# faasm/faabric

Hardware: AMD Instinct MI355X
Metric: MPI_Allreduce GB/s + batch-exec msgs/sec, 8-rank world at 1/2/4/8 MI355X (higher is better)
Workload: dtype fp32; 1 GPU; model=faabric composite: 256MB fp32 allreduce + 1MB alltoall + kvtouch batch, global_batch=128, parallelism=mpi1, allreduce_bytes=268435456, pingpong_bytes=0, kv_bytes=4096, full=False, snapshot_bytes_per_rank=0, snapshot_dirty=random-scattered 25pct, random-byte region, gpu=True

## Files before the change

### cpp/bindings/bindings_runtime.cpp

```cpp
#include <pybind11/functional.h>
#include <pybind11/pybind11.h>
#include <pybind11/stl.h>

#include "faabricamd/endpoint.h"
#include "faabricamd/executor.h"
#include "faabricamd/flat.h"
#include "faabricamd/hipipc.h"
#include "faabricamd/planner.h"
#include "faabricamd/ptp.h"
#include "faabricamd/runner.h"
#include "faabricamd/scheduler.h"
#include "faabricamd/snapshot.h"
#include "faabricamd/state.h"
#include "faabricamd/util.h"
#include "faabricamd/utilextras.h"
#include "faabricamd/dirty.h"
#include <hip/hip_runtime.h>

namespace py = pybind11;
using namespace faabricamd;

namespace faabricamd {
void registerBenchFunctions();
std::map<std::string, std::vector<uint8_t>> benchLastOutputs();
// ... 794 lines not shown
            PageAlignedBuffer buf;
            buf.resize(16 * 4096);
            tracker.startTracking(buf.data(), buf.size());
            buf.data()[2 * 4096 + 11] = 42;
            buf.data()[14 * 4096] = 7;
            tracker.stopTracking(buf.data(), buf.size());
            auto dirty = tracker.getDirtyPages(buf.data(), buf.size());
            int nDirty = 0;
            for (char d : dirty) {
                nDirty += d != 0;
            }
            ok = nDirty == 2 && dirty[2] == 1 && dirty[14] == 1;
        }
        return py::bool_(ok);
    });

    m.def("_selftest_softpte_tracker", []() -> py::object {
        if (!SoftPTEDirtyTracker::isAvailable()) {
            return py::none();
        }
        bool ok;
        {
            py::gil_scoped_release release;
            SoftPTEDirtyTracker tracker;
            PageAlignedBuffer buf;
            buf.resize(16 * 4096);
            std::memset(buf.data(), 1, buf.size());
            tracker.startTracking(buf.data(), buf.size());
            buf.data()[5 * 4096 + 3] = 42;
            buf.data()[12 * 4096] = 7;
            tracker.stopTracking(buf.data(), buf.size());
            auto dirty = tracker.getDirtyPages(buf.data(), buf.size());
            ok = dirty.size() == 16 && dirty[5] == 1 && dirty[12] == 1;
        }
        return py::bool_(ok);
    });

    m.def("_debug_runtime_sizes", [] {
        py::dict d;
        d["planner_app_results"] = Planner::get().debugAppResultsCount();
        d["planner_done_apps"] = Planner::get().debugDoneAppsCount();
        d["planner_in_flight"] = Planner::get().debugInFlightCount();
        d["broker_mappings"] = getPointToPointBroker().debugMappingsCount();
        d["broker_channels"] = getPointToPointBroker().debugChannelsCount();
        d["broker_send_seqs"] = getPointToPointBroker().debugSendSeqsCount();
        d["decision_cache"] = DecisionCache::get().size();
        return d;
    });
    m.def("_debug_dispatch_sizes", [] {
        py::dict d;
        d["idle_executors"] = Scheduler::get().debugIdleCount();
        d["planner_msg_index_apps"] = Planner::get().debugMsgIndexCount();
        d["planner_used_slots"] = Planner::get().debugUsedSlots();
        return d;
    });
    m.def("_debug_current_executor_id", [] {
        return ExecutorContext::get().getExecutor()->id;
    });
    m.def("_debug_set_message_result", [](const Message& msg) {
        auto copy = std::make_shared<Message>(msg);
        py::gil_scoped_release release;
        getPlannerClient().setMessageResult(copy);
    });
    m.def("_debug_kv_commit_stats", [] {
        KvCommitStats s = kvCommitStats();
        py::dict d;
        d["launches"] = s.launches;
        d["pages"] = s.pages;
        return d;
    });
    m.def("_debug_kv_sweep_bitmap",
          [](size_t nPages, const std::vector<uint64_t>& setBits) {
              size_t nWords = (nPages + 63) / 64;
              auto words = std::make_unique<std::atomic<uint64_t>[]>(
                std::max<size_t>(nWords, 1));
              for (size_t w = 0; w < nWords; w++) {
                  words[w].store(0);
              }
              for (uint64_t b : setBits) {
                  if (b >= nPages) {
                      throw FaabricException("bit beyond the bitmap");
                  }
                  words[b / 64].fetch_or(1ULL << (b % 64));
              }
              std::vector<uint32_t> pages(nPages);
              size_t n =
                kvSweepDirtyBitmap(words.get(), nPages, pages.data());
              pages.resize(n);
              std::vector<uint64_t> after(nWords);
              for (size_t w = 0; w < nWords; w++) {
                  after[w] = words[w].load();
              }
              return py::make_tuple(pages, after);
          },
          py::arg("n_pages"),
          py::arg("set_bits"));
    m.def("wait_batch_done",
          [](int32_t appId, int timeoutMs) {
              py::gil_scoped_release release;
              return getPlannerClient().waitBatchDone(appId, timeoutMs);
          },
          py::arg("app_id"),
          py::arg("timeout_ms") = 30000);
    m.def("set_bound_timeout",
          [](int ms) { getSystemConfig().boundTimeout = ms; });
    m.def("reap_stale_executors", [] {
        py::gil_scoped_release release;
        return Scheduler::get().reapStaleExecutors();
    });
    m.def("register_bench_functions", [] { registerBenchFunctions(); });
    m.def("bench_last_outputs", [] {
        py::dict d;
        for (const auto& [name, data] : benchLastOutputs()) {
            d[py::str(name)] =
              py::bytes((const char*)data.data(), data.size());
        }
        return d;
    });
    m.def("register_mpi_example_functions",
          [] { registerMpiExampleFunctions(); });

    m.def("execute_threads",
          [](const std::string& user,
             const std::string& function,
             int nThreads,
             const std::vector<std::tuple<uint32_t, size_t, int, int>>&
               regions,
             const py::bytes& inputData,
             bool elastic) {
              Executor* exec = ExecutorContext::get().getExecutor();
              std::string input = inputData;
              std::vector<std::pair<int32_t, int32_t>> results;
              {
                  py::gil_scoped_release release;
                  auto req = std::make_shared<BatchExecuteRequest>(
                    batchExecFactory(user, function, nThreads));
                  req->elasticScaleHint = elastic;
                  for (auto& m2 : req->messages) {
                      m2.inputData.assign(input.begin(), input.end());
                  }
                  std::vector<SnapshotMergeRegion> mr;
                  for (const auto& [off, len, dt, op] : regions) {
                      mr.emplace_back(off,
                                      len,
                                      (SnapshotDataType)dt,
                                      (SnapshotMergeOperation)op);
                  }
                  results = exec->executeThreads(req, mr);
              }
              py::list out;
              for (auto& [msgId, rv] : results) {
                  out.append(py::make_tuple(msgId, rv));
              }
              return out;
          },
          py::arg("user"),
          py::arg("function"),
          py::arg("n_threads"),
// ... 123 lines not shown
```

### cpp/include/faabricamd/executor.h

```cpp
#pragma once

#include <atomic>
#include <functional>
#include <memory>
#include <string>
#include <thread>
#include <vector>

#include "faabricamd/mailbox.h"
#include "faabricamd/messages.h"
#include "faabricamd/queue.h"
#include "faabricamd/dirty.h"
#include "faabricamd/snapshot.h"

namespace faabricamd {

class Executor;


class ExecutorContext
{
  public:
    static bool isSet();
    static void set(Executor* executor,
// ... 64 lines not shown
    std::vector<std::pair<int32_t, int32_t>> executeThreads(
      std::shared_ptr<BatchExecuteRequest> req,
      const std::vector<SnapshotMergeRegion>& mergeRegions);

    virtual int32_t executeTask(int threadPoolIdx,
                                int msgIdx,
                                std::shared_ptr<BatchExecuteRequest> req);

    virtual std::pair<uint8_t*, size_t> getMemoryView();
    virtual void setMemorySize(size_t newSize);
    void setDeviceMemorySize(size_t newSize);
    std::pair<uint8_t*, size_t> getDeviceMemoryView();
    bool hasDeviceArena() const { return deviceArena != nullptr; }
    virtual void restore(const std::string& snapshotKey);
    virtual void reset(Message& msg);
    virtual void flush();

    bool tryClaim();
    void claim();
    void releaseClaim();
    bool isClaimed() const { return claimed.load(); }
    using IdleExecutors = IdleList<std::shared_ptr<Executor>>;
    void setIdleList(std::shared_ptr<IdleExecutors> list)
    {
        idleList = std::move(list);
    }

    long getMillisSinceLastExec() const;
    void shutdown();

    std::string id;
    Message boundMsg;
    int gpuDevice = -1;

    void setThreadResult(Message& msg,
                         int32_t returnValue,
                         const std::string& key,
                         const std::vector<SnapshotDiffMsg>& diffs);

  protected:
    void threadPoolThread(int poolIdx);
    void handleTaskResult(Message& msg,
                          int32_t returnValue,
                          std::shared_ptr<BatchExecuteRequest> req,
                          bool isLastInBatch);

    int threadPoolSize = 0;
    using TaskMailbox = Mailbox<ExecutorTask>;
    std::vector<std::unique_ptr<TaskMailbox>> threadMailboxes;
    std::vector<std::thread> threadPoolThreads;
    std::unique_ptr<std::atomic<bool>[]> poolThreadUp;
    std::mutex threadsMx;
    void ensurePoolThreadLocked(int poolIdx);
    void postTask(int poolIdx, ExecutorTask&& task);

    std::shared_ptr<IdleExecutors> idleList;

    std::atomic<bool> claimed{ false };
    std::atomic<int64_t> lastExecMs{ 0 };

    std::string lastForkSnapshotKey;
    std::vector<std::string> lastForkRemoteHosts;
    void cleanupForkSnapshot();

    std::shared_ptr<std::atomic<int>> batchCounter;

    PageAlignedBuffer dummyMemory;

    uint8_t* deviceArena = nullptr;
    size_t deviceArenaSize = 0;
};

class ExecutorFactory
{
  public:
    virtual ~ExecutorFactory() = default;
    virtual std::shared_ptr<Executor> createExecutor(Message& msg)
    {
        return std::make_shared<Executor>(msg);
    }
    virtual void flushHost() {}
};

void setExecutorFactory(std::shared_ptr<ExecutorFactory> factory);
std::shared_ptr<ExecutorFactory> getExecutorFactory();

int32_t chainFunction(const std::string& user,
                      const std::string& function,
                      const std::vector<uint8_t>& input);
Message awaitChainedCall(int32_t msgId, int timeoutMs = 60000);

int32_t migrationPoint(const std::vector<uint8_t>& reentryInput);

}
```

### cpp/include/faabricamd/mailbox.h

```cpp
#pragma once

#include <atomic>
#include <climits>
#include <cstddef>
#include <cstdint>
#include <ctime>
#include <mutex>
#include <utility>
#include <vector>

#include <linux/futex.h>
#include <sys/syscall.h>
#include <unistd.h>

namespace faabricamd {

namespace detail {

inline void futexWait(std::atomic<uint32_t>* word,
                      uint32_t expected,
                      int timeoutMs)
{
    static_assert(sizeof(std::atomic<uint32_t>) == sizeof(uint32_t));
    struct timespec ts;
    struct timespec* tsp = nullptr;
    if (timeoutMs > 0) {
        ts.tv_sec = timeoutMs / 1000;
        ts.tv_nsec = (long)(timeoutMs % 1000) * 1000000L;
        tsp = &ts;
    }
    syscall(SYS_futex,
            reinterpret_cast<uint32_t*>(word),
            FUTEX_WAIT_PRIVATE,
            expected,
            tsp,
            nullptr,
            0);
}

inline void futexWake(std::atomic<uint32_t>* word, int n)
{
    syscall(SYS_futex,
            reinterpret_cast<uint32_t*>(word),
            FUTEX_WAKE_PRIVATE,
            n,
            nullptr,
            nullptr,
            0);
}

}

template<typename T, uint32_t SLOTS = 8>
class Mailbox
{
    static_assert(SLOTS >= 2 && (SLOTS & (SLOTS - 1)) == 0,
                  "SLOTS must be a power of two");

  public:
    Mailbox()
    {
        for (uint32_t i = 0; i < SLOTS; i++) {
            slots[i].seq.store(i, std::memory_order_relaxed);
        }
    }
    Mailbox(const Mailbox&) = delete;
    Mailbox& operator=(const Mailbox&) = delete;

    void post(T value)
    {
        uint32_t ticket = tail.fetch_add(1, std::memory_order_relaxed);
        Slot& s = slots[ticket & (SLOTS - 1)];
        uint32_t seen;
        while ((seen = s.seq.load(std::memory_order_acquire)) != ticket) {
            detail::futexWait(&s.seq, seen, 1);
        }
        s.value = std::move(value);
        s.seq.store(ticket + 1, std::memory_order_seq_cst);
        if (sleeping.load(std::memory_order_seq_cst) != 0) {
            detail::futexWake(&s.seq, INT_MAX);
        }
    }

    bool take(T& out, int timeoutMs)
    {
        Slot& s = slots[head & (SLOTS - 1)];
        uint32_t ready = head + 1;
        uint32_t seen = s.seq.load(std::memory_order_acquire);
        if (seen != ready) {
            struct timespec start;
            clock_gettime(CLOCK_MONOTONIC, &start);
            int leftMs = timeoutMs;
            while (true) {
                sleeping.store(1, std::memory_order_seq_cst);
                seen = s.seq.load(std::memory_order_seq_cst);
                if (seen != ready) {
                    detail::futexWait(&s.seq, seen, leftMs);
                    seen = s.seq.load(std::memory_order_acquire);
                }
                sleeping.store(0, std::memory_order_relaxed);
                if (seen == ready) {
                    break;
                }
                if (timeoutMs > 0) {
                    struct timespec now;
                    clock_gettime(CLOCK_MONOTONIC, &now);
                    int64_t goneMs =
                      (int64_t)(now.tv_sec - start.tv_sec) * 1000 +
                      (now.tv_nsec - start.tv_nsec) / 1000000;
                    if (goneMs >= timeoutMs) {
                        return false;
                    }
                    leftMs = (int)(timeoutMs - goneMs);
                }
            }
        }
        out = std::move(s.value);
        s.value = T();
        s.seq.store(head + SLOTS, std::memory_order_release);
        head++;
        return true;
    }

  private:
    struct alignas(64) Slot
    {
        std::atomic<uint32_t> seq{ 0 };
        T value{};
    };
    Slot slots[SLOTS];
    alignas(64) std::atomic<uint32_t> tail{ 0 };
    std::atomic<uint32_t> sleeping{ 0 };
    alignas(64) uint32_t head = 0;
};

template<typename T>
class IdleList
{
  public:
    void push(T value)
    {
        std::lock_guard<std::mutex> lock(mx);
        if (!closed) {
            entries.push_back(std::move(value));
        }
    }

    size_t popMany(size_t n, std::vector<T>& out)
    {
        std::lock_guard<std::mutex> lock(mx);
        size_t got = 0;
        while (got < n && !entries.empty()) {
            out.push_back(std::move(entries.back()));
            entries.pop_back();
            got++;
        }
        return got;
    }

    bool pop(T& out)
    {
        std::lock_guard<std::mutex> lock(mx);
        if (entries.empty()) {
            return false;
        }
        out = std::move(entries.back());
        entries.pop_back();
        return true;
    }

    size_t remove(const T& value)
    {
        std::lock_guard<std::mutex> lock(mx);
        size_t before = entries.size();
        size_t w = 0;
        for (size_t r = 0; r < entries.size(); r++) {
            if (!(entries[r] == value)) {
                if (w != r) {
                    entries[w] = std::move(entries[r]);
                }
                w++;
            }
        }
        entries.resize(w);
        return before - w;
    }

    void close()
    {
        std::vector<T> dropped;
        {
            std::lock_guard<std::mutex> lock(mx);
            closed = true;
            dropped.swap(entries);
        }
    }

    size_t size()
    {
        std::lock_guard<std::mutex> lock(mx);
        return entries.size();
    }

  private:
    std::mutex mx;
    std::vector<T> entries;
    bool closed = false;
};

}
```

### cpp/include/faabricamd/scheduler.h

```cpp
#pragma once

#include <memory>
#include <mutex>
#include <shared_mutex>
#include <unordered_map>
#include <vector>

#include "faabricamd/executor.h"
#include "faabricamd/messages.h"
#include "faabricamd/queue.h"
#include "faabricamd/transport.h"

namespace faabricamd {

enum class FunctionCalls : uint8_t
{
    ExecuteFunctions = 1,
    Flush = 2,
    SetMessageResult = 3,
    BatchDone = 4,
};

class Scheduler
{
  public:
    static Scheduler& get();

    void executeBatch(std::shared_ptr<BatchExecuteRequest> req);

    HostResources getThisHostResources();
    void setThisHostResources(const HostResources& res);

    int reapStaleExecutors();
    void startReaper();
    void stopReaper();

    std::shared_ptr<PendingMigration> checkForMigrationOpportunities(
      Message& msg,
      int32_t overwriteNewGroupId = 0);

    void flushLocally();
    void shutdown();
    void reset();

    std::vector<Message> getRecordedMessages();
    void clearRecordedMessages();

    size_t getExecutorCount();
    size_t debugIdleCount();

  private:
    Scheduler();

    struct WarmPool
    {
        std::vector<std::shared_ptr<Executor>> list;
        std::shared_ptr<Executor::IdleExecutors> idle =
          std::make_shared<Executor::IdleExecutors>();
    };

    std::shared_ptr<Executor> claimExecutor(Message& msg);
    void claimExecutors(BatchExecuteRequest& req,
                        std::vector<std::shared_ptr<Executor>>& execs,
                        std::vector<std::string>& errors);
    std::shared_ptr<Executor> createExecutorLocked(WarmPool& pool,
                                                   Message& msg);

    std::shared_mutex schedMx;
    std::unordered_map<std::string, std::unique_ptr<WarmPool>> executors;
    HostResources overriddenResources;
    bool resourcesOverridden = false;

    std::vector<Message> recordedMessages;

    class ReaperThread;
    std::shared_ptr<ReaperThread> reaper;
};

bool functionCallServerRunning();

class FunctionCallServer : public MessageEndpointServer
{
  public:
    FunctionCallServer();
    ~FunctionCallServer() override;
    void doAsyncRecv(uint8_t code,
                     const std::string& body,
                     uint32_t seq) override;
    std::string doSyncRecv(uint8_t code, const std::string& body) override;
};

class FunctionCallClient : public MessageEndpointClient
{
  public:
    explicit FunctionCallClient(const std::string& host);
    void executeFunctions(const BatchExecuteRequest& req);
    void setMessageResult(const Message& msg);
    void sendFlush();
    void batchDone(int32_t appId);
};

std::shared_ptr<FunctionCallClient> getFunctionCallClient(
  const std::string& host);

std::shared_ptr<FlagWaiter> batchDoneWaiterPrepare(int32_t appId);
void batchDoneWaiterDiscard(int32_t appId);
void signalBatchDone(int32_t appId);
void clearFunctionCallClients();

std::vector<std::pair<std::string, BatchExecuteRequest>>
getBatchRequestsSentMock();
void clearMockedFunctionCalls();

}
```

### cpp/src/executor.cpp

```cpp
#include "faabricamd/executor.h"
#include "faabricamd/utilextras.h"
#include "faabricamd/mpi.h"
#include "faabricamd/ops.h"
#include "faabricamd/planner.h"

#include <hip/hip_runtime.h>
#include "faabricamd/snapshot.h"
#include "faabricamd/util.h"

#include <algorithm>
#include <cstring>

namespace faabricamd {

void resultBatcherEnqueue(std::shared_ptr<Message> msg);


static thread_local std::shared_ptr<ExecutorContext> currentContext;

bool ExecutorContext::isSet()
{
    return currentContext != nullptr;
}

void ExecutorContext::set(Executor* executor,
                          std::shared_ptr<BatchExecuteRequest> req,
                          int msgIdx)
{
    auto ctx = std::make_shared<ExecutorContext>();
    ctx->executor = executor;
    ctx->req = std::move(req);
    ctx->msgIdx = msgIdx;
    currentContext = ctx;
}

void ExecutorContext::unset()
{
    currentContext = nullptr;
}

ExecutorContext& ExecutorContext::get()
{
    if (!currentContext) {
        throw FaabricException("no executor context set");
    }
    return *currentContext;
}

Message& ExecutorContext::getMsg()
{
    return req->messages.at(msgIdx);
}


FunctionRegistry& FunctionRegistry::get()
{
    static FunctionRegistry reg;
    return reg;
}

void FunctionRegistry::registerFunction(const std::string& user,
                                        const std::string& function,
                                        FaabricFunction fn)
{
    std::lock_guard<std::mutex> lock(mx);
    functions[user + "/" + function] = std::move(fn);
}

// ... 96 lines not shown
    std::lock_guard<std::mutex> lock(threadsMx);
    for (int i = 0; i < threadPoolSize; i++) {
        if (threadPoolThreads[i].joinable()) {
            ExecutorTask stopTask;
            stopTask.stop = true;
            threadMailboxes[i]->post(std::move(stopTask));
        }
    }
    for (int i = 0; i < threadPoolSize; i++) {
        if (threadPoolThreads[i].joinable()) {
            threadPoolThreads[i].join();
            poolThreadUp[i].store(false, std::memory_order_release);
        }
    }
}

long Executor::getMillisSinceLastExec() const
{
    return (long)(getGlobalClockEpochMillis() - lastExecMs.load());
}

bool Executor::tryClaim()
{
    bool expected = false;
    return claimed.compare_exchange_strong(expected, true);
}

void Executor::claim()
{
    claimed.store(true);
}

void Executor::releaseClaim()
{
    claimed.store(false);
    if (idleList) {
        idleList->push(shared_from_this());
    }
}

void Executor::ensurePoolThreadLocked(int poolIdx)
{
    if (threadPoolThreads[poolIdx].joinable()) {
        return;
    }
    if (!threadMailboxes[poolIdx]) {
        threadMailboxes[poolIdx] = std::make_unique<TaskMailbox>();
    }
    threadPoolThreads[poolIdx] =
      std::thread([this, poolIdx] { threadPoolThread(poolIdx); });
    poolThreadUp[poolIdx].store(true, std::memory_order_release);
}

void Executor::postTask(int poolIdx, ExecutorTask&& task)
{
    task.enqueueNs = profEnabled() ? profNowNs() : 0;
    threadMailboxes[poolIdx]->post(std::move(task));
}

void Executor::executeSingleTask(
  int msgIdx,
  const std::shared_ptr<BatchExecuteRequest>& req)
{
    if (req->type == BatchExecuteType::THREADS ||
        !req->snapshotKey.empty() ||
        !req->messages.at(msgIdx).snapshotKey.empty() ||
        threadPoolSize == 0) {
        executeTasks({ msgIdx }, req);
        return;
    }
    lastExecMs = getGlobalClockEpochMillis();
    if (!poolThreadUp[0].load(std::memory_order_acquire)) {
        std::lock_guard<std::mutex> lock(threadsMx);
        ensurePoolThreadLocked(0);
    }
    ExecutorTask task(msgIdx, req);
    task.single = true;
    postTask(0, std::move(task));
}

void Executor::executeTasks(const std::vector<int>& msgIdxs,
                            const std::shared_ptr<BatchExecuteRequest>& req)
{
    lastExecMs = getGlobalClockEpochMillis();
    batchCounter = std::make_shared<std::atomic<int>>((int)msgIdxs.size());

    if (!req->snapshotKey.empty()) {
        restore(req->snapshotKey);
    } else if (!req->messages.empty() &&
               !req->messages[msgIdxs[0]].snapshotKey.empty() &&
               req->type != BatchExecuteType::THREADS) {
        const std::string& key = req->messages[msgIdxs[0]].snapshotKey;
        restore(key);
        if (startsWith(key, "migration_")) {
            SnapshotRegistry::get().deleteSnapshot(key);
            DeviceSnapshotRegistry::get().deleteSnapshot(key);
        }
    }

    if (req->type == BatchExecuteType::THREADS &&
        !req->snapshotKey.empty()) {
        auto tracker = getDirtyTracker();
        if (tracker->getType() == "segfault") {
            auto [base, size] = getMemoryView();
            if (size > 0) {
                tracker->startTracking(base, size);
            }
        }
    }

    std::lock_guard<std::mutex> lock(threadsMx);
    for (int msgIdx : msgIdxs) {
        int poolIdx = threadPoolSize == 0 ? 0 : msgIdx % threadPoolSize;
        ensurePoolThreadLocked(poolIdx);
        postTask(poolIdx, ExecutorTask(msgIdx, req));
    }
}

std::vector<std::pair<int32_t, int32_t>> Executor::executeThreads(
  std::shared_ptr<BatchExecuteRequest> req,
  const std::vector<SnapshotMergeRegion>& mergeRegions)
{
    Message& parentMsg = ExecutorContext::get().getMsg();
    std::string key = getMainThreadSnapshotKey(
      parentMsg.user, parentMsg.function, parentMsg.appId);

    bool onDevice = hasDeviceArena();
    {
        Message& pm = ExecutorContext::get().getMsg();
        std::string newKey = getMainThreadSnapshotKey(
          pm.user, pm.function, pm.appId);
// ... 148 lines not shown
            if (deviceArenaSize < dsnap->size()) {
                setDeviceMemorySize(dsnap->size());
            }
            hipError_t err = hipMemcpy(deviceArena,
                                       dsnap->data(),
                                       dsnap->size(),
                                       hipMemcpyDeviceToDevice);
            if (err != hipSuccess ||
                hipStreamSynchronize(nullptr) != hipSuccess) {
                throw FaabricException("device snapshot restore failed");
            }
            return;
        }
        if (SnapshotRegistry::get().snapshotExists(snapshotKey)) {
            auto snap = SnapshotRegistry::get().getSnapshot(snapshotKey);
            if (dummyMemory.size() < snap->getSize()) {
                setMemorySize(snap->getSize());
            }
            auto [base, size] = getMemoryView();
            snap->mapToMemory(base, size);
            return;
        }
        if (getGlobalClockEpochMillis() >= deadline) {
            throw FaabricException("snapshot not found: " + snapshotKey);
        }
        usleep(10 * 1000);
    }
}

void Executor::reset(Message& msg)
{
    (void)msg;
}

void Executor::flush()
{
    FunctionRegistry::get().clear();
}

void Executor::setThreadResult(Message& msg,
                               int32_t returnValue,
                               const std::string& key,
                               const std::vector<SnapshotDiffMsg>& diffs)
{
    (void)key;
    (void)diffs;
    msg.returnValue = returnValue;
}

void Executor::threadPoolThread(int poolIdx)
{
    const auto& conf = getSystemConfig();
    TaskMailbox& mailbox = *threadMailboxes[poolIdx];
    while (true) {
        ExecutorTask task;
        if (!mailbox.take(task, conf.boundTimeout)) {
            continue;
        }
        if (task.stop) {
            break;
        }
        if (task.enqueueNs != 0) {
            profRecord("exec_wake",
                       (double)(profNowNs() - task.enqueueNs) / 1e6);
        }

        Message& msg = task.req->messages.at(task.msgIdx);
        int32_t returnValue = 0;
        ExecutorContext::set(this, task.req, task.msgIdx);
        try {
            PROF_START(exec_task)
            returnValue = executeTask(poolIdx, task.msgIdx, task.req);
            PROF_END(exec_task)
            if (msg.isMpi && msg.recordExecGraph &&
                MpiWorldRegistry::get().worldExists(msg.mpiWorldId)) {
                auto counts = MpiWorldRegistry::get()
                                .getWorld(msg.mpiWorldId)
                                .getMsgCountDetails(msg.mpiRank);
                for (const auto& [k, v] : counts) {
                    msg.intExecGraphDetails[k] = v;
                }
            }
        } catch (const FunctionMigratedException&) {
            FAM_DEBUG("task %d migrated", msg.id);
            returnValue = MIGRATED_FUNCTION_RETURN_VALUE;
        } catch (const FunctionFrozenException&) {
            FAM_DEBUG("task %d frozen", msg.id);
            returnValue = FROZEN_FUNCTION_RETURN_VALUE;
        } catch (const std::exception& e) {
            FAM_ERROR("task %d failed: %s", msg.id, e.what());
            returnValue = 1;
            msg.outputData = std::string("Task failed: ") + e.what();
        }
        ExecutorContext::unset();

        bool isLastInBatch =
          task.single || batchCounter->fetch_sub(1) - 1 == 0;
        handleTaskResult(msg, returnValue, task.req, isLastInBatch);
    }
}

void Executor::handleTaskResult(Message& msg,
                                int32_t returnValue,
                                std::shared_ptr<BatchExecuteRequest> req,
                                bool isLastInBatch)
{
    const auto& conf = getSystemConfig();
    msg.returnValue = returnValue;
    msg.executedHost = conf.endpointHost;
    msg.finishTimestamp = getGlobalClockEpochMillis();
    lastExecMs = getGlobalClockEpochMillis();

    bool isThreads = req->type == BatchExecuteType::THREADS;

// ... 50 lines not shown
                auto dirty = tracker->getDirtyPages(base, size);
                threadDiffs =
                  snap->diffWithDirtyRegions(base, size, dirty);
            } else {
                threadDiffs = snap->diffWithMemory(base, size);
            }
        } catch (const std::exception& e) {
            FAM_ERROR("thread diff failed: %s", e.what());
        }
    }

    if (isLastInBatch) {
        if (!isThreads) {
            try {
                reset(msg);
            } catch (const std::exception& e) {
                FAM_ERROR("executor reset failed: %s", e.what());
            }
        }
        releaseClaim();
    }

    if (isThreads && !req->snapshotKey.empty()) {
        const std::string& mainHost = msg.mainHost;
        if (mainHost == conf.endpointHost || mainHost.empty()) {
            if (!threadDiffs.empty()) {
                try {
                    if (deviceThreads) {
                        auto dsnap = DeviceSnapshotRegistry::get()
                                       .getSnapshot(req->snapshotKey);
                        for (auto& d : threadDiffs) {
                            dsnap->queuePackedDiff(d.dataCopy);
                        }
                    } else {
                        auto snap = SnapshotRegistry::get().getSnapshot(
                          req->snapshotKey);
                        snap->queueDiffs(threadDiffs);
                    }
                } catch (const std::exception& e) {
                    FAM_ERROR("queueing thread diffs failed: %s", e.what());
                }
            }
            auto resultMsg = std::make_shared<Message>(msg);
            PROF_START(result_rpc)
            getPlannerClient().setMessageResult(resultMsg);
            PROF_END(result_rpc)
        } else {
            getSnapshotClient(mainHost)->pushThreadResult(
              msg.appId, msg.id, returnValue, req->snapshotKey, threadDiffs);
        }
        return;
    }

    resultBatcherEnqueue(std::make_shared<Message>(msg));
}


namespace {

struct ResultBatcher
{
    std::mutex mx;
    std::condition_variable cv;
    std::vector<std::shared_ptr<Message>> queue;
    std::thread worker;
    bool stop = false;
    bool started = false;

    void ensureStarted()
    {
        std::lock_guard<std::mutex> lock(mx);
        if (started) {
            return;
        }
        started = true;
        worker = std::thread([this] { run(); });
    }

    void run()
    {
        std::vector<std::shared_ptr<Message>> batch;
        while (true) {
            {
                std::unique_lock<std::mutex> lock(mx);
                cv.wait(lock, [&] { return stop || !queue.empty(); });
                if (stop && queue.empty()) {
                    return;
                }
                batch.swap(queue);
            }
            try {
                PROF_START(result_batch_send)
                getPlannerClient().setMessageResultsBatch(batch);
                PROF_END(result_batch_send)
            } catch (const std::exception& e) {
                FAM_ERROR("result batch send failed: %s", e.what());
            }
            batch.clear();
        }
    }

    ~ResultBatcher()
    {
        {
            std::lock_guard<std::mutex> lock(mx);
            stop = true;
        }
// ... 75 lines not shown
```

### cpp/src/scheduler.cpp

```cpp
#include "faabricamd/scheduler.h"
#include "faabricamd/utilextras.h"

#include <atomic>
#include <thread>
#include <functional>
#include <condition_variable>
#include "faabricamd/planner.h"
#include "faabricamd/ptp.h"
#include "faabricamd/util.h"
#include "faabricamd/wire.h"

#include <hip/hip_runtime.h>

namespace faabricamd {

static int getNumGpus()
{
    static int n = []() {
        const auto& conf = getSystemConfig();
        if (conf.overrideGpuCount >= 0) {
            return conf.overrideGpuCount;
        }
        if (!conf.useGpu) {
            return 0;
        }
        int count = 0;
        if (hipGetDeviceCount(&count) != hipSuccess) {
            return 0;
        }
        return count;
    }();
    return n;
}

class Scheduler::ReaperThread : public PeriodicBackgroundThread
{
  public:
    void doWork() override { Scheduler::get().reapStaleExecutors(); }
};

Scheduler::Scheduler() = default;

Scheduler& Scheduler::get()
{
    static Scheduler sched;
    return sched;
}

HostResources Scheduler::getThisHostResources()
{
    {
        std::unique_lock<std::shared_mutex> lock(schedMx);
        if (resourcesOverridden) {
            return overriddenResources;
        }
    }
    HostResources res;
    int nGpus = getNumGpus();
    res.slots = nGpus > 0 ? nGpus : getUsableCores();
    res.usedSlots = 0;
    return res;
}

void Scheduler::setThisHostResources(const HostResources& res)
{
    std::unique_lock<std::shared_mutex> lock(schedMx);
    overriddenResources = res;
    resourcesOverridden = true;
}

void Scheduler::executeBatch(std::shared_ptr<BatchExecuteRequest> req)
{
    if (req->messages.empty()) {
        return;
    }
    PROF_START(sched_execute_batch)
    bool isThreads = req->type == BatchExecuteType::THREADS;

    if (isTestMode()) {
        std::unique_lock<std::shared_mutex> lock(schedMx);
        for (const auto& msg : req->messages) {
            recordedMessages.push_back(msg);
        }
    }

    if (isThreads) {
        auto exec = claimExecutor(req->messages[0]);
        std::vector<int> idxs(req->messages.size());
        for (size_t i = 0; i < idxs.size(); i++) {
            idxs[i] = (int)i;
        }
        exec->executeTasks(idxs, req);
    } else {
        size_t n = req->messages.size();
        std::vector<std::shared_ptr<Executor>> execs;
        std::vector<std::string> claimErrors;
        PROF_START(dispatch_claim)
        claimExecutors(*req, execs, claimErrors);
        PROF_END(dispatch_claim)

        PROF_START(dispatch_enqueue)
        for (size_t i = 0; i < n; i++) {
            try {
                if (!execs[i]) {
                    throw FaabricException(claimErrors[i]);
                }
                execs[i]->executeSingleTask((int)i, req);
            } catch (const std::exception& e) {
                FAM_ERROR("claiming executor failed: %s", e.what());
                if (execs[i]) {
                    execs[i]->releaseClaim();
                }
                auto msg = std::make_shared<Message>(req->messages[i]);
                msg->returnValue = 1;
                msg->executedHost = getSystemConfig().endpointHost;
                msg->outputData = std::string("executor claim failed: ") +
                                  e.what();
                getPlannerClient().setMessageResult(msg);
            }
        }
        PROF_END(dispatch_enqueue)
    }
    PROF_END(sched_execute_batch)
}

static std::shared_ptr<Executor> popIdleClaimed(
  Executor::IdleExecutors& idle)
{
    std::shared_ptr<Executor> e;
    while (idle.pop(e)) {
        if (e->tryClaim()) {
            return e;
        }
    }
    return nullptr;
}

std::shared_ptr<Executor> Scheduler::createExecutorLocked(WarmPool& pool,
                                                          Message& msg)
{
    auto exec = getExecutorFactory()->createExecutor(msg);
    exec->claim();
    exec->setIdleList(pool.idle);
    if (getNumGpus() > 0) {
        const auto& conf = getSystemConfig();
        exec->gpuDevice =
          conf.gpuDevicePinned
            ? conf.gpuDevice
            : (int)((pool.list.size()) % (size_t)getNumGpus());
    }
    pool.list.push_back(exec);
    return exec;
}

std::shared_ptr<Executor> Scheduler::claimExecutor(Message& msg)
{
    std::string key = msg.user + "/" + msg.function;

    {
        std::shared_lock<std::shared_mutex> rlock(schedMx);
        auto it = executors.find(key);
        if (it != executors.end()) {
            if (auto e = popIdleClaimed(*it->second->idle)) {
                return e;
            }
        }
    }

    std::unique_lock<std::shared_mutex> lock(schedMx);
    auto& poolPtr = executors[key];
    if (!poolPtr) {
        poolPtr = std::make_unique<WarmPool>();
    }
    if (auto e = popIdleClaimed(*poolPtr->idle)) {
        return e;
    }
    return createExecutorLocked(*poolPtr, msg);
}

void Scheduler::claimExecutors(
  BatchExecuteRequest& req,
  std::vector<std::shared_ptr<Executor>>& execs,
  std::vector<std::string>& errors)
{
    size_t n = req.messages.size();
    execs.assign(n, nullptr);
    errors.assign(n, std::string());

    const Message& first = req.messages[0];
    bool oneFunction = true;
    for (size_t i = 1; i < n && oneFunction; i++) {
        oneFunction = req.messages[i].function == first.function &&
                      req.messages[i].user == first.user;
    }
    if (!oneFunction) {
        for (size_t i = 0; i < n; i++) {
            try {
                execs[i] = claimExecutor(req.messages[i]);
            } catch (const std::exception& e) {
                errors[i] = e.what();
            }
        }
        return;
    }

    std::string key = first.user + "/" + first.function;
    std::vector<std::shared_ptr<Executor>> popped;
    popped.reserve(n);
    size_t got = 0;
    auto takeIdle = [&](Executor::IdleExecutors& idle) {
        while (got < n) {
            popped.clear();
            if (idle.popMany(n - got, popped) == 0) {
                return;
            }
            for (auto& e : popped) {
                if (e->tryClaim()) {
                    execs[got++] = std::move(e);
                }
            }
        }
    };
    {
        std::shared_lock<std::shared_mutex> rlock(schedMx);
        auto it = executors.find(key);
        if (it != executors.end()) {
            takeIdle(*it->second->idle);
        }
    }
    if (got == n) {
        return;
    }

    std::unique_lock<std::shared_mutex> lock(schedMx);
    auto& poolPtr = executors[key];
    if (!poolPtr) {
        poolPtr = std::make_unique<WarmPool>();
    }
    takeIdle(*poolPtr->idle);
    poolPtr->list.reserve(poolPtr->list.size() + (n - got));
    for (; got < n; got++) {
        try {
            execs[got] = createExecutorLocked(*poolPtr, req.messages[got]);
        } catch (const std::exception& e) {
            errors[got] = e.what();
        }
    }
}

int Scheduler::reapStaleExecutors()
{
    std::unique_lock<std::shared_mutex> lock(schedMx);
    const auto& conf = getSystemConfig();
    int reaped = 0;
    for (auto& [key, pool] : executors) {
        auto& list = pool->list;
        for (auto it = list.begin(); it != list.end();) {
            auto& exec = *it;
            if (exec->getMillisSinceLastExec() > conf.boundTimeout &&
                exec->tryClaim()) {
                pool->idle->remove(exec);
                exec->shutdown();
                it = list.erase(it);
                reaped++;
            } else {
                ++it;
            }
        }
    }
    return reaped;
}

void Scheduler::startReaper()
{
    if (!reaper) {
        reaper = std::make_shared<ReaperThread>();
        reaper->startMillis(getSystemConfig().boundTimeout);
    }
}

void Scheduler::stopReaper()
{
    if (reaper) {
        reaper->stop();
        reaper = nullptr;
    }
}

std::shared_ptr<PendingMigration> Scheduler::checkForMigrationOpportunities(
  Message& msg,
  int32_t overwriteNewGroupId)
{
    int32_t newGroupId = 0;
    if (msg.groupIdx == 0 && overwriteNewGroupId == 0) {
        auto req = std::make_shared<BatchExecuteRequest>();
        req->appId = msg.appId;
        req->groupId = msg.groupId;
        req->user = msg.user;
        req->function = msg.function;
        req->type = BatchExecuteType::MIGRATION;
// ... 64 lines not shown
void Scheduler::shutdown()
{
    stopReaper();
    std::unique_lock<std::shared_mutex> lock(schedMx);
    for (auto& [key, pool] : executors) {
        pool->idle->close();
        for (auto& e : pool->list) {
            e->shutdown();
        }
    }
    executors.clear();
}

void Scheduler::reset()
{
    shutdown();
    std::unique_lock<std::shared_mutex> lock(schedMx);
    recordedMessages.clear();
    resourcesOverridden = false;
}

std::vector<Message> Scheduler::getRecordedMessages()
{
    std::unique_lock<std::shared_mutex> lock(schedMx);
    return recordedMessages;
}

void Scheduler::clearRecordedMessages()
{
    std::unique_lock<std::shared_mutex> lock(schedMx);
    recordedMessages.clear();
}

size_t Scheduler::getExecutorCount()
{
    std::unique_lock<std::shared_mutex> lock(schedMx);
    size_t n = 0;
    for (auto& [key, pool] : executors) {
        n += pool->list.size();
    }
    return n;
}

size_t Scheduler::debugIdleCount()
{
    std::shared_lock<std::shared_mutex> lock(schedMx);
    size_t n = 0;
    for (auto& [key, pool] : executors) {
        n += pool->idle->size();
    }
    return n;
}


static std::atomic<int> fnServersUp{ 0 };

bool functionCallServerRunning()
{
    return fnServersUp.load(std::memory_order_relaxed) > 0;
}

FunctionCallServer::FunctionCallServer()
  : MessageEndpointServer(FUNCTION_CALL_ASYNC_PORT,
                          FUNCTION_CALL_SYNC_PORT,
                          "function-call")
{
    fnServersUp.fetch_add(1, std::memory_order_relaxed);
}

FunctionCallServer::~FunctionCallServer()
{
    fnServersUp.fetch_sub(1, std::memory_order_relaxed);
}


static std::mutex batchDoneMx;
static std::map<int32_t, std::shared_ptr<FlagWaiter>> batchDoneFlags;

std::shared_ptr<FlagWaiter> batchDoneWaiterPrepare(int32_t appId)
{
    std::lock_guard<std::mutex> lock(batchDoneMx);
    auto& w = batchDoneFlags[appId];
    if (!w) {
        w = std::make_shared<FlagWaiter>();
    }
    return w;
}

void batchDoneWaiterDiscard(int32_t appId)
{
    std::lock_guard<std::mutex> lock(batchDoneMx);
    batchDoneFlags.erase(appId);
}

void signalBatchDone(int32_t appId)
{
    std::shared_ptr<FlagWaiter> w;
    {
        std::lock_guard<std::mutex> lock(batchDoneMx);
        auto it = batchDoneFlags.find(appId);
        if (it == batchDoneFlags.end()) {
            return;
        }
        w = it->second;
    }
    w->setFlag(true);
// ... 132 lines not shown
```

Before: 200,200 msgs/sec.

## Claim executors lazily per message, prefer oldest idle, add optional spin-before-park

Batch dispatch stops claiming all executors up front. It now pre-grows the warm pool and pops one idle executor per message while enqueueing. When spinning is off it takes the oldest idle executor first, and the idle list becomes a deque to support that. Pool threads can spin briefly before parking on the futex while a batch is dispatching, though the spin is disabled by default (budget 0). Non-thread results now share ownership with the request instead of copying the message. Together these aim to cut futex wake latency and per-message allocation, at the cost of more complex claim logic and possible CPU burn when spinning is enabled.

```diff
diff --git a/cpp/bindings/bindings_runtime.cpp b/cpp/bindings/bindings_runtime.cpp
--- a/cpp/bindings/bindings_runtime.cpp
+++ b/cpp/bindings/bindings_runtime.cpp
@@ -870,6 +870,12 @@
         d["idle_executors"] = Scheduler::get().debugIdleCount();
         d["planner_msg_index_apps"] = Planner::get().debugMsgIndexCount();
         d["planner_used_slots"] = Planner::get().debugUsedSlots();
+        d["spinning_threads"] = Scheduler::get().debugSpinningThreads();
+        d["dispatching_batches"] =
+          Scheduler::get().debugDispatchingBatches();
+        HandoffCounts handoffs = getHandoffCounts();
+        d["handoffs_without_wake"] = handoffs.withoutWake;
+        d["handoffs_with_wake"] = handoffs.withWake;
         return d;
     });
     m.def("_debug_current_executor_id", [] {
@@ -922,6 +928,14 @@
           py::arg("timeout_ms") = 30000);
     m.def("set_bound_timeout",
           [](int ms) { getSystemConfig().boundTimeout = ms; });
+    m.def("set_executor_spin",
+          [](int budgetUs, int maxSpinners) {
+              setExecutorSpin(budgetUs, maxSpinners);
+              return py::make_tuple(getExecutorSpinUs(),
+                                    getExecutorSpinners());
+          },
+          py::arg("budget_us"),
+          py::arg("max_spinners") = -1);
     m.def("reap_stale_executors", [] {
         py::gil_scoped_release release;
         return Scheduler::get().reapStaleExecutors();
diff --git a/cpp/include/faabricamd/executor.h b/cpp/include/faabricamd/executor.h
--- a/cpp/include/faabricamd/executor.h
+++ b/cpp/include/faabricamd/executor.h
@@ -140,7 +140,7 @@
     std::unique_ptr<std::atomic<bool>[]> poolThreadUp;
     std::mutex threadsMx;
     void ensurePoolThreadLocked(int poolIdx);
-    void postTask(int poolIdx, ExecutorTask&& task);
+    bool postTask(int poolIdx, ExecutorTask&& task);
 
     std::shared_ptr<IdleExecutors> idleList;
 
@@ -170,6 +170,17 @@
     virtual void flushHost() {}
 };
 
+void setExecutorSpin(int budgetUs, int maxSpinners);
+int getExecutorSpinUs();
+int getExecutorSpinners();
+
+struct HandoffCounts
+{
+    uint64_t withoutWake = 0;
+    uint64_t withWake = 0;
+};
+HandoffCounts getHandoffCounts();
+
 void setExecutorFactory(std::shared_ptr<ExecutorFactory> factory);
 std::shared_ptr<ExecutorFactory> getExecutorFactory();
 
diff --git a/cpp/include/faabricamd/mailbox.h b/cpp/include/faabricamd/mailbox.h
--- a/cpp/include/faabricamd/mailbox.h
+++ b/cpp/include/faabricamd/mailbox.h
@@ -4,7 +4,9 @@
 #include <climits>
 #include <cstddef>
 #include <cstdint>
+#include <deque>
 #include <ctime>
+#include <iterator>
 #include <mutex>
 #include <utility>
 #include <vector>
@@ -49,7 +51,29 @@
             0);
 }
 
-}
+inline void cpuRelax()
+{
+#if defined(__x86_64__) || defined(__i386__)
+    __builtin_ia32_pause();
+#elif defined(__aarch64__)
+    asm volatile("yield" ::: "memory");
+#endif
+}
+
+}
+
+struct SpinGate
+{
+    alignas(64) std::atomic<int> dispatching{ 0 };
+    alignas(64) std::atomic<int> spinning{ 0 };
+};
+
+struct SpinBeforePark
+{
+    SpinGate* gate = nullptr;
+    int budgetUs = 0;
+    int maxSpinners = 0;
+};
 
 template<typename T, uint32_t SLOTS = 8>
 class Mailbox
@@ -67,7 +91,7 @@
     Mailbox(const Mailbox&) = delete;
     Mailbox& operator=(const Mailbox&) = delete;
 
-    void post(T value)
+    bool post(T value)
     {
         uint32_t ticket = tail.fetch_add(1, std::memory_order_relaxed);
         Slot& s = slots[ticket & (SLOTS - 1)];
@@ -79,14 +103,19 @@
         s.seq.store(ticket + 1, std::memory_order_seq_cst);
         if (sleeping.load(std::memory_order_seq_cst) != 0) {
             detail::futexWake(&s.seq, INT_MAX);
-        }
-    }
-
-    bool take(T& out, int timeoutMs)
+            return true;
+        }
+        return false;
+    }
+
+    bool take(T& out, int timeoutMs, const SpinBeforePark* spin = nullptr)
     {
         Slot& s = slots[head & (SLOTS - 1)];
         uint32_t ready = head + 1;
         uint32_t seen = s.seq.load(std::memory_order_acquire);
+        if (seen != ready && spin != nullptr) {
+            seen = spinFor(s, ready, *spin);
+        }
         if (seen != ready) {
             struct timespec start;
             clock_gettime(CLOCK_MONOTONIC, &start);
@@ -128,6 +157,45 @@
         std::atomic<uint32_t> seq{ 0 };
         T value{};
     };
+
+    uint32_t spinFor(Slot& s, uint32_t ready, const SpinBeforePark& spin)
+    {
+        uint32_t seen = s.seq.load(std::memory_order_acquire);
+        SpinGate* gate = spin.gate;
+        if (gate == nullptr || spin.budgetUs <= 0 ||
+            gate->dispatching.load(std::memory_order_relaxed) <= 0) {
+            return seen;
+        }
+        if (gate->spinning.fetch_add(1, std::memory_order_relaxed) >=
+            spin.maxSpinners) {
+            gate->spinning.fetch_sub(1, std::memory_order_relaxed);
+            return seen;
+        }
+        struct timespec start;
+        clock_gettime(CLOCK_MONOTONIC, &start);
+        int64_t budgetNs = (int64_t)spin.budgetUs * 1000;
+        while (true) {
+            for (int i = 0; i < 32 && seen != ready; i++) {
+                detail::cpuRelax();
+                seen = s.seq.load(std::memory_order_acquire);
+            }
+            if (seen == ready ||
+                gate->dispatching.load(std::memory_order_relaxed) <= 0) {
+                break;
+            }
+            struct timespec now;
+            clock_gettime(CLOCK_MONOTONIC, &now);
+            int64_t goneNs =
+              (int64_t)(now.tv_sec - start.tv_sec) * 1000000000LL +
+              (now.tv_nsec - start.tv_nsec);
+            if (goneNs >= budgetNs) {
+                break;
+            }
+        }
+        gate->spinning.fetch_sub(1, std::memory_order_relaxed);
+        return seen;
+    }
+
     Slot slots[SLOTS];
     alignas(64) std::atomic<uint32_t> tail{ 0 };
     std::atomic<uint32_t> sleeping{ 0 };
@@ -146,6 +214,16 @@
         }
     }
 
+    void pushBottom(std::vector<T>& values)
+    {
+        std::lock_guard<std::mutex> lock(mx);
+        if (!closed) {
+            entries.insert(entries.begin(),
+                           std::make_move_iterator(values.begin()),
+                           std::make_move_iterator(values.end()));
+        }
+    }
+
     size_t popMany(size_t n, std::vector<T>& out)
     {
         std::lock_guard<std::mutex> lock(mx);
@@ -166,6 +244,17 @@
         }
         out = std::move(entries.back());
         entries.pop_back();
+        return true;
+    }
+
+    bool popOldest(T& out)
+    {
+        std::lock_guard<std::mutex> lock(mx);
+        if (entries.empty()) {
+            return false;
+        }
+        out = std::move(entries.front());
+        entries.pop_front();
         return true;
     }
 
@@ -188,7 +277,7 @@
 
     void close()
     {
-        std::vector<T> dropped;
+        std::deque<T> dropped;
         {
             std::lock_guard<std::mutex> lock(mx);
             closed = true;
@@ -202,9 +291,11 @@
         return entries.size();
     }
 
+    SpinGate gate;
+
   private:
     std::mutex mx;
-    std::vector<T> entries;
+    std::deque<T> entries;
     bool closed = false;
 };
 
diff --git a/cpp/include/faabricamd/scheduler.h b/cpp/include/faabricamd/scheduler.h
--- a/cpp/include/faabricamd/scheduler.h
+++ b/cpp/include/faabricamd/scheduler.h
@@ -48,6 +48,8 @@
 
     size_t getExecutorCount();
     size_t debugIdleCount();
+    int debugSpinningThreads();
+    int debugDispatchingBatches();
 
   private:
     Scheduler();
@@ -60,11 +62,11 @@
     };
 
     std::shared_ptr<Executor> claimExecutor(Message& msg);
-    void claimExecutors(BatchExecuteRequest& req,
-                        std::vector<std::shared_ptr<Executor>>& execs,
-                        std::vector<std::string>& errors);
+    std::shared_ptr<Executor::IdleExecutors> prepareWarmPool(Message& msg,
+                                                             size_t n);
     std::shared_ptr<Executor> createExecutorLocked(WarmPool& pool,
-                                                   Message& msg);
+                                                   Message& msg,
+                                                   bool claimed = true);
 
     std::shared_mutex schedMx;
     std::unordered_map<std::string, std::unique_ptr<WarmPool>> executors;
diff --git a/cpp/src/executor.cpp b/cpp/src/executor.cpp
--- a/cpp/src/executor.cpp
+++ b/cpp/src/executor.cpp
@@ -14,6 +14,40 @@
 namespace faabricamd {
 
 void resultBatcherEnqueue(std::shared_ptr<Message> msg);
+
+static std::atomic<int> execSpinUs{ getEnvVarInt("FAABRIC_EXEC_SPIN_US", 0) };
+static std::atomic<int> execSpinners{ getEnvVarInt("FAABRIC_EXEC_SPINNERS",
+                                                   4) };
+static std::atomic<uint64_t> handoffsWithoutWake{ 0 };
+static std::atomic<uint64_t> handoffsWithWake{ 0 };
+
+void setExecutorSpin(int budgetUs, int maxSpinners)
+{
+    if (budgetUs >= 0) {
+        execSpinUs.store(budgetUs, std::memory_order_relaxed);
+    }
+    if (maxSpinners >= 0) {
+        execSpinners.store(maxSpinners, std::memory_order_relaxed);
+    }
+}
+
+int getExecutorSpinUs()
+{
+    return execSpinUs.load(std::memory_order_relaxed);
+}
+
+int getExecutorSpinners()
+{
+    return execSpinners.load(std::memory_order_relaxed);
+}
+
+HandoffCounts getHandoffCounts()
+{
+    HandoffCounts c;
+    c.withoutWake = handoffsWithoutWake.load(std::memory_order_relaxed);
+    c.withWake = handoffsWithWake.load(std::memory_order_relaxed);
+    return c;
+}
 
 
 static thread_local std::shared_ptr<ExecutorContext> currentContext;
@@ -216,10 +250,10 @@
     poolThreadUp[poolIdx].store(true, std::memory_order_release);
 }
 
-void Executor::postTask(int poolIdx, ExecutorTask&& task)
+bool Executor::postTask(int poolIdx, ExecutorTask&& task)
 {
     task.enqueueNs = profEnabled() ? profNowNs() : 0;
-    threadMailboxes[poolIdx]->post(std::move(task));
+    return threadMailboxes[poolIdx]->post(std::move(task));
 }
 
 void Executor::executeSingleTask(
@@ -240,7 +274,9 @@
     }
     ExecutorTask task(msgIdx, req);
     task.single = true;
-    postTask(0, std::move(task));
+    bool woke = postTask(0, std::move(task));
+    (woke ? handoffsWithWake : handoffsWithoutWake)
+      .fetch_add(1, std::memory_order_relaxed);
 }
 
 void Executor::executeTasks(const std::vector<int>& msgIdxs,
@@ -495,14 +531,25 @@
 {
     const auto& conf = getSystemConfig();
     TaskMailbox& mailbox = *threadMailboxes[poolIdx];
+    bool afterSingle = false;
     while (true) {
         ExecutorTask task;
-        if (!mailbox.take(task, conf.boundTimeout)) {
+        SpinBeforePark spin;
+        if (afterSingle && idleList) {
+            spin.gate = &idleList->gate;
+            spin.budgetUs = getExecutorSpinUs();
+            spin.maxSpinners = getExecutorSpinners();
+        }
+        afterSingle = false;
+        if (!mailbox.take(task,
+                          conf.boundTimeout,
+                          spin.gate != nullptr ? &spin : nullptr)) {
             continue;
         }
         if (task.stop) {
             break;
         }
+        afterSingle = task.single;
         if (task.enqueueNs != 0) {
             profRecord("exec_wake",
                        (double)(profNowNs() - task.enqueueNs) / 1e6);
@@ -659,7 +706,11 @@
         return;
     }
 
-    resultBatcherEnqueue(std::make_shared<Message>(msg));
+    if (isThreads) {
+        resultBatcherEnqueue(std::make_shared<Message>(msg));
+    } else {
+        resultBatcherEnqueue(std::shared_ptr<Message>(req, &msg));
+    }
 }
 
 
diff --git a/cpp/src/scheduler.cpp b/cpp/src/scheduler.cpp
--- a/cpp/src/scheduler.cpp
+++ b/cpp/src/scheduler.cpp
@@ -69,6 +69,19 @@
     resourcesOverridden = true;
 }
 
+static std::shared_ptr<Executor> popIdleClaimed(
+  Executor::IdleExecutors& idle,
+  bool oldestFirst = false)
+{
+    std::shared_ptr<Executor> e;
+    while (oldestFirst ? idle.popOldest(e) : idle.pop(e)) {
+        if (e->tryClaim()) {
+            return e;
+        }
+    }
+    return nullptr;
+}
+
 void Scheduler::executeBatch(std::shared_ptr<BatchExecuteRequest> req)
 {
     if (req->messages.empty()) {
@@ -93,30 +106,60 @@
         exec->executeTasks(idxs, req);
     } else {
         size_t n = req->messages.size();
-        std::vector<std::shared_ptr<Executor>> execs;
-        std::vector<std::string> claimErrors;
         PROF_START(dispatch_claim)
-        claimExecutors(*req, execs, claimErrors);
+        std::shared_ptr<Executor::IdleExecutors> idle;
+        try {
+            idle = prepareWarmPool(req->messages[0], n);
+        } catch (const std::exception& e) {
+            FAM_ERROR("growing the warm pool failed: %s", e.what());
+        }
         PROF_END(dispatch_claim)
+        const Message& first = req->messages[0];
+
+        struct DispatchScope
+        {
+            SpinGate* gate;
+            explicit DispatchScope(SpinGate* g)
+              : gate(g)
+            {
+                if (gate) {
+                    gate->dispatching.fetch_add(1, std::memory_order_relaxed);
+                }
+            }
+            ~DispatchScope()
+            {
+                if (gate) {
+                    gate->dispatching.fetch_sub(1, std::memory_order_relaxed);
+                }
+            }
+        } dispatching(idle ? &idle->gate : nullptr);
+
+        bool oldestFirst = getExecutorSpinUs() <= 0;
 
         PROF_START(dispatch_enqueue)
         for (size_t i = 0; i < n; i++) {
+            Message& msg = req->messages[i];
+            std::shared_ptr<Executor> exec;
             try {
-                if (!execs[i]) {
-                    throw FaabricException(claimErrors[i]);
+                if (idle && (i == 0 || (msg.function == first.function &&
+                                        msg.user == first.user))) {
+                    exec = popIdleClaimed(*idle, oldestFirst);
                 }
-                execs[i]->executeSingleTask((int)i, req);
+                if (!exec) {
+                    exec = claimExecutor(msg);
+                }
+                exec->executeSingleTask((int)i, req);
             } catch (const std::exception& e) {
                 FAM_ERROR("claiming executor failed: %s", e.what());
-                if (execs[i]) {
-                    execs[i]->releaseClaim();
+                if (exec) {
+                    exec->releaseClaim();
                 }
-                auto msg = std::make_shared<Message>(req->messages[i]);
-                msg->returnValue = 1;
-                msg->executedHost = getSystemConfig().endpointHost;
-                msg->outputData = std::string("executor claim failed: ") +
-                                  e.what();
-                getPlannerClient().setMessageResult(msg);
+                auto errMsg = std::make_shared<Message>(msg);
+                errMsg->returnValue = 1;
+                errMsg->executedHost = getSystemConfig().endpointHost;
+                errMsg->outputData =
+                  std::string("executor claim failed: ") + e.what();
+                getPlannerClient().setMessageResult(errMsg);
             }
         }
         PROF_END(dispatch_enqueue)
@@ -124,23 +167,14 @@
     PROF_END(sched_execute_batch)
 }
 
-static std::shared_ptr<Executor> popIdleClaimed(
-  Executor::IdleExecutors& idle)
-{
-    std::shared_ptr<Executor> e;
-    while (idle.pop(e)) {
-        if (e->tryClaim()) {
-            return e;
-        }
-    }
-    return nullptr;
-}
-
 std::shared_ptr<Executor> Scheduler::createExecutorLocked(WarmPool& pool,
-                                                          Message& msg)
+                                                          Message& msg,
+                                                          bool claimed)
 {
     auto exec = getExecutorFactory()->createExecutor(msg);
-    exec->claim();
+    if (claimed) {
+        exec->claim();
+    }
     exec->setIdleList(pool.idle);
     if (getNumGpus() > 0) {
         const auto& conf = getSystemConfig();
@@ -178,58 +212,17 @@
     return createExecutorLocked(*poolPtr, msg);
 }
 
-void Scheduler::claimExecutors(
-  BatchExecuteRequest& req,
-  std::vector<std::shared_ptr<Executor>>& execs,
-  std::vector<std::string>& errors)
-{
-    size_t n = req.messages.size();
-    execs.assign(n, nullptr);
-    errors.assign(n, std::string());
-
-    const Message& first = req.messages[0];
-    bool oneFunction = true;
-    for (size_t i = 1; i < n && oneFunction; i++) {
-        oneFunction = req.messages[i].function == first.function &&
-                      req.messages[i].user == first.user;
-    }
-    if (!oneFunction) {
-        for (size_t i = 0; i < n; i++) {
-            try {
-                execs[i] = claimExecutor(req.messages[i]);
-            } catch (const std::exception& e) {
-                errors[i] = e.what();
-            }
-        }
-        return;
-    }
-
-    std::string key = first.user + "/" + first.function;
-    std::vector<std::shared_ptr<Executor>> popped;
-    popped.reserve(n);
-    size_t got = 0;
-    auto takeIdle = [&](Executor::IdleExecutors& idle) {
-        while (got < n) {
-            popped.clear();
-            if (idle.popMany(n - got, popped) == 0) {
-                return;
-            }
-            for (auto& e : popped) {
-                if (e->tryClaim()) {
-                    execs[got++] = std::move(e);
-                }
-            }
-        }
-    };
+std::shared_ptr<Executor::IdleExecutors> Scheduler::prepareWarmPool(
+  Message& msg,
+  size_t n)
+{
+    std::string key = msg.user + "/" + msg.function;
     {
         std::shared_lock<std::shared_mutex> rlock(schedMx);
         auto it = executors.find(key);
-        if (it != executors.end()) {
-            takeIdle(*it->second->idle);
-        }
-    }
-    if (got == n) {
-        return;
+        if (it != executors.end() && it->second->idle->size() >= n) {
+            return it->second->idle;
+        }
     }
 
     std::unique_lock<std::shared_mutex> lock(schedMx);
@@ -237,15 +230,23 @@
     if (!poolPtr) {
         poolPtr = std::make_unique<WarmPool>();
     }
-    takeIdle(*poolPtr->idle);
-    poolPtr->list.reserve(poolPtr->list.size() + (n - got));
-    for (; got < n; got++) {
+    WarmPool& pool = *poolPtr;
+    size_t have = pool.idle->size();
+    if (have < n) {
+        std::vector<std::shared_ptr<Executor>> fresh;
+        fresh.reserve(n - have);
+        pool.list.reserve(pool.list.size() + (n - have));
         try {
-            execs[got] = createExecutorLocked(*poolPtr, req.messages[got]);
-        } catch (const std::exception& e) {
-            errors[got] = e.what();
-        }
-    }
+            for (size_t i = have; i < n; i++) {
+                fresh.push_back(createExecutorLocked(pool, msg, false));
+            }
+        } catch (...) {
+            pool.idle->pushBottom(fresh);
+            throw;
+        }
+        pool.idle->pushBottom(fresh);
+    }
+    return pool.idle;
 }
 
 int Scheduler::reapStaleExecutors()
@@ -416,6 +417,26 @@
     return n;
 }
 
+int Scheduler::debugSpinningThreads()
+{
+    std::shared_lock<std::shared_mutex> lock(schedMx);
+    int n = 0;
+    for (auto& [key, pool] : executors) {
+        n += pool->idle->gate.spinning.load(std::memory_order_relaxed);
+    }
+    return n;
+}
+
+int Scheduler::debugDispatchingBatches()
+{
+    std::shared_lock<std::shared_mutex> lock(schedMx);
+    int n = 0;
+    for (auto& [key, pool] : executors) {
+        n += pool->idle->gate.dispatching.load(std::memory_order_relaxed);
+    }
+    return n;
+}
+
 
 static std::atomic<int> fnServersUp{ 0 };
 
```

Measured after the change: 165,800 msgs/sec. 0.828x the previous value.
